# ToniChopp/ECAMP

Hardware: AMD Instinct MI355X
Metric: pretrain image-report pairs/sec (ViT-B/16, 224^2, seq=128) (higher is better)
Workload: dtype bf16

## Files before the change

### ecamp_amd/csrc/vision.hip

```cpp
#include "common.h"
#include <stdlib.h>
#include <stdint.h>

__device__ __forceinline__ void cubic_coeffs(float t, float (&w)[4]) {
    const float A = -0.75f;
    float x;
    x = t + 1.0f; w[0] = ((A * x - 5.0f * A) * x + 8.0f * A) * x - 4.0f * A;
    x = t;        w[1] = ((A + 2.0f) * x - (A + 3.0f)) * x * x + 1.0f;
    x = 1.0f - t; w[2] = ((A + 2.0f) * x - (A + 3.0f)) * x * x + 1.0f;
    x = 2.0f - t; w[3] = ((A * x - 5.0f * A) * x + 8.0f * A) * x - 4.0f * A;
}
__global__ void bicubic_kernel(const float* __restrict__ src, float* __restrict__ dst, long planes, int Hs, int Ws, int Hd,
                               int Wd, float sy, float sx) {
    long n = planes * Hd * Wd;
    for (long i = (long)blockIdx.x * blockDim.x + threadIdx.x; i < n; i += (long)gridDim.x * blockDim.x) {
        int x = (int)(i % Wd), y = (int)((i / Wd) % Hd);
        long pl = i / ((long)Wd * Hd);
        float ry = sy * (y + 0.5f) - 0.5f, rx = sx * (x + 0.5f) - 0.5f;
        float fy = floorf(ry), fx = floorf(rx);
        float wy[4], wx[4];
        cubic_coeffs(ry - fy, wy);
        cubic_coeffs(rx - fx, wx);
        int iy = (int)fy, ix = (int)fx;
        const float* p = src + pl * (long)Hs * Ws;
// ... 997 lines not shown
            for (int e = 0; e < 2; ++e) {
                u32x4_t q;
                q[0] = in ? pack_bf16x2(o[0][e][0], o[1][e][0]) : 0u;
                q[1] = in ? pack_bf16x2(o[2][e][0], 0.f) : 0u;
                q[2] = in ? pack_bf16x2(o[0][e][1], o[1][e][1]) : 0u;
                q[3] = in ? pack_bf16x2(o[2][e][1], 0.f) : 0u;
                *reinterpret_cast<u32x4_t*>(U16 + ((2 * by + e) * 36 + 2 * bx) * 8) = q;
            }
            if (by >= 1 && by <= 16 && bx >= 1 && bx <= 16) {
#pragma unroll
                for (int c = 0; c < 3; ++c)
#pragma unroll
                    for (int e = 0; e < 2; ++e)
                        *reinterpret_cast<float2*>(UC + (c * 32 + 2 * by - 2 + e) * 32 + 2 * bx - 2) = make_float2(o[c][e][0], o[c][e][1]);
            }
        }
        __syncthreads();
        for (int g = wave; g < (34 * 17 + 63) / 64; g += 4) {
            const int p = g * 64 + lane, pc = min(p, 34 * 17 - 1);
            const int y = pc / 17, xq = pc - y * 17;
            f32x4_t oA, oB;
            sr_pair_conv<36, false>(U16 + (y * 36 + 2 * xq) * 8, a1, bias1, oA, oB);
            const int Y = Y0 - 1 + y, X = X0 - 1 + 2 * xq;
            const bool iy = Y >= 0 && Y < R2, inA = iy && X >= 0 && X < R2, inB = iy && X + 1 >= 0 && X + 1 < R2;
            u32x4_t q;
            q[0] = inA ? pack_bf16x2(fmaxf(oA[0], 0.f), fmaxf(oA[1], 0.f)) : 0u;
            q[1] = inA ? pack_bf16x2(fmaxf(oA[2], 0.f), 0.f) : 0u;
            q[2] = inB ? pack_bf16x2(fmaxf(oB[0], 0.f), fmaxf(oB[1], 0.f)) : 0u;
            q[3] = inB ? pack_bf16x2(fmaxf(oB[2], 0.f), 0.f) : 0u;
            if (p < 34 * 17) *reinterpret_cast<u32x4_t*>(C16 + (y * 34 + 2 * xq) * 8) = q;
        }
        __syncthreads();
#pragma unroll
        for (int j = 0; j < 2; ++j) {
            const int p = (wave + 4 * j) * 64 + lane, y = p >> 4, xq = p & 15;
            float2 bg[3];
#pragma unroll
            for (int o = 0; o < 3; ++o) bg[o] = big.at2(b, o, Y0 + y, X0 + 2 * xq, R2);
            f32x4_t oA, oB;
            sr_pair_conv<34, false>(C16 + (y * 34 + 2 * xq) * 8, a2, bias2, oA, oB);
#pragma unroll
            for (int o = 0; o < 3; ++o) {
                const float2 uu = *reinterpret_cast<const float2*>(UC + (o * 32 + y) * 32 + 2 * xq);
                const float dA = fmaxf(oA[o] + uu.x, 0.f) - bg[o].x, dB = fmaxf(oB[o] + uu.y, 0.f) - bg[o].y;
                part += dA * dA + dB * dB;
            }
        }
    }
    part = block_sum_256(part, sh);
    if (threadIdx.x == 0) atomicAdd(loss_sum, part);
}

#define SRP_LDS_BYTES (44 * 44 * 8 + 40 * 42 * 8 + 38 * 40 * 8 + 36 * 38 * 8 + 3 * 34 * 36 * 4 + 4 * 9 * 4 * 8)
__global__ __launch_bounds__(256, 2) void sr_pair_bwd_kernel(const float* __restrict__ pred_img, BigSrc big,
                                                             const long* __restrict__ column, const long* __restrict__ row, SrP P,
                                                             float* __restrict__ dsr, float* __restrict__ gw, long B, int R, int win) {
    extern __shared__ __attribute__((aligned(16))) unsigned char smem8[];
    unsigned char* U16 = smem8;
    unsigned char* C16 = U16 + 44 * 44 * 8;
    unsigned char* DS16 = C16 + 40 * 42 * 8;
    unsigned char* DC16 = DS16 + 38 * 40 * 8;
    float* DU = reinterpret_cast<float*>(DC16 + 36 * 38 * 8);
    float* PP = DU;
    bf16x4_t(*TAPS)[9][4] = reinterpret_cast<bf16x4_t(*)[9][4]>(reinterpret_cast<unsigned char*>(DU) + 3 * 34 * 36 * 4);
    const int lane = threadIdx.x & 63, wave = threadIdx.x >> 6;
    if (threadIdx.x < 144) {
        const int c = threadIdx.x / 36, t = (threadIdx.x / 4) % 9, i = threadIdx.x & 3;
        const float* w = (c == 0 || c == 3) ? P.w1 : P.w2;
        const bool trans = c >= 2;
        float v[3] = {0.f, 0.f, 0.f};
        if (i < 3) {
            for (int kk = 0; kk < 3; ++kk) v[kk] = trans ? w[(kk * 3 + i) * 9 + t] : w[(i * 3 + kk) * 9 + t];
        }
        TAPS[c][t][i] = sr_pack4(v[0], v[1], v[2]);
    }
#define SR_TAPS(NAME, C)                                                     \
    bf16x4_t NAME[9];                                                        \
    _Pragma("unroll") for (int t_ = 0; t_ < 9; ++t_) NAME[t_] = TAPS[(C)][t_][lane & 3]
    const f32x4_t bias1 = {P.b1[0], P.b1[1], P.b1[2], 0.f}, bias2 = {P.b2[0], P.b2[1], P.b2[2], 0.f}, zero4 = {0.f, 0.f, 0.f, 0.f};
    const bf16x4_t ones = {(short)H16_ONE, (short)H16_ONE, (short)H16_ONE, (short)H16_ONE};
    const int R2 = 2 * R, G = R2 / SRT, PT = SRT / 2;
    const long T = B * G * G;
    f32x4_t G1[9], G2[9], gb1 = zero4, gb2 = zero4;
#pragma unroll
    for (int q = 0; q < 9; ++q) G1[q] = G2[q] = zero4;
    const int py = threadIdx.x / PT, px = threadIdx.x % PT;

    struct Cur { int t, b, ty, tx; };
    const int GG = G * G, NT = (int)T;
    const int step_b = (int)gridDim.x / GG, step_r = (int)gridDim.x - step_b * GG, step_y = step_r / G, step_x = step_r - step_y * G;
    auto step = [&](Cur c) {
        c.t += (int)gridDim.x;
        c.tx += step_x;
        if (c.tx >= G) { c.tx -= G; ++c.ty; }
        c.ty += step_y;
        if (c.ty >= G) { c.ty -= G; ++c.b; }
        c.b += step_b;
        return c;
    };
    auto advance = [&](Cur c) {
        for (; c.t < NT; c = step(c)) {
            const int c0 = (int)column[c.b], r0 = (int)row[c.b];
            if (!(c.ty < c0 - 1 || c.ty > c0 + win || c.tx < r0 - 1 || c.tx > r0 + win)) break;
#pragma unroll
            for (int ch = 0; ch < 3; ++ch) dsr[((c.b * 3 + ch) * (long)R + c.ty * PT + py) * R + c.tx * PT + px] = 0.f;
        }
        return c;
    };
    float pp[7], bigv[3][3][2];
    bool inw[3];
    auto fetch_patch = [&](const Cur& cu) {
        const long b = cu.b;
        const int ylo = cu.ty * (SRT / 2) - 4, xlo = cu.tx * (SRT / 2) - 4;
#pragma unroll
        for (int k = 0; k < 7; ++k) {
            const int idx = threadIdx.x + 256 * k;
// ... 25 lines not shown
            }
        }
    };
    Cur cur;
    cur.t = (int)blockIdx.x; cur.b = cur.t / GG; cur.ty = (cur.t - cur.b * GG) / G; cur.tx = cur.t - cur.b * GG - cur.ty * G;
    cur = advance(cur);
    if (cur.t < NT) {
        fetch_patch(cur);
        fetch_big(cur);
    }
    while (cur.t < NT) {
        const long b = cur.b;
        const int ty = cur.ty, tx = cur.tx;
        const int Y0 = ty * SRT, X0 = tx * SRT;
        __syncthreads();
#pragma unroll
        for (int k = 0; k < 7; ++k) {
            const int idx = threadIdx.x + 256 * k;
            if (idx < 3 * 576) PP[idx] = pp[k];
        }
        const Cur nxt = advance(step(cur));
        if (nxt.t < NT) fetch_patch(nxt);
        __syncthreads();
        for (int id = threadIdx.x; id < 22 * 22; id += 256) {
            const int by = id / 22, bx = id - by * 22;
            float o[3][2][2];
#pragma unroll
            for (int c = 0; c < 3; ++c) {
                const float* pl = PP + c * 576 + by * 24 + bx;
                float he[3], ho[3];
#pragma unroll
                for (int r = 0; r < 3; ++r) {
                    const float v0 = pl[r * 24], v1 = pl[r * 24 + 1], v2 = pl[r * 24 + 2];
                    he[r] = 0.25f * v0 + 0.75f * v1;
                    ho[r] = 0.75f * v1 + 0.25f * v2;
                }
                o[c][0][0] = 0.25f * he[0] + 0.75f * he[1];
                o[c][0][1] = 0.25f * ho[0] + 0.75f * ho[1];
                o[c][1][0] = 0.75f * he[1] + 0.25f * he[2];
                o[c][1][1] = 0.75f * ho[1] + 0.25f * ho[2];
            }
            const int Y = Y0 - 6 + 2 * by, X = X0 - 6 + 2 * bx;
            const bool in = Y >= 0 && Y < R2 && X >= 0 && X < R2;
#pragma unroll
            for (int e = 0; e < 2; ++e) {
                u32x4_t q;
                q[0] = in ? pack_bf16x2(o[0][e][0], o[1][e][0]) : 0u;
                q[1] = in ? pack_bf16x2(o[2][e][0], 0.f) : 0u;
                q[2] = in ? pack_bf16x2(o[0][e][1], o[1][e][1]) : 0u;
                q[3] = in ? pack_bf16x2(o[2][e][1], 0.f) : 0u;
                *reinterpret_cast<u32x4_t*>(U16 + ((2 * by + e) * 44 + 2 * bx) * 8) = q;
            }
        }
        __syncthreads();
        {
            SR_TAPS(a1, 0);
            for (int g = wave; g < (40 * 21 + 63) / 64; g += 4) {
                const int p = g * 64 + lane, pc = min(p, 40 * 21 - 1);
                const int y = pc / 21, xq = pc - y * 21;
                f32x4_t oA, oB;
                sr_pair_conv<44, false>(U16 + ((y + 1) * 44 + 2 * xq) * 8, a1, bias1, oA, oB);
                const int Y = Y0 - 4 + y, X = X0 - 5 + 2 * xq;
                const bool iy = Y >= 0 && Y < R2, inA = iy && X >= 0 && X < R2, inB = iy && X + 1 >= 0 && X + 1 < R2;
                u32x4_t q;
                q[0] = inA ? pack_bf16x2(fmaxf(oA[0], 0.f), fmaxf(oA[1], 0.f)) : 0u;
                q[1] = inA ? pack_bf16x2(fmaxf(oA[2], 0.f), 0.f) : 0u;
                q[2] = inB ? pack_bf16x2(fmaxf(oB[0], 0.f), fmaxf(oB[1], 0.f)) : 0u;
                q[3] = inB ? pack_bf16x2(fmaxf(oB[2], 0.f), 0.f) : 0u;
                if (p < 40 * 21) *reinterpret_cast<u32x4_t*>(C16 + (y * 42 + 2 * xq) * 8) = q;
            }
        }
        __syncthreads();
        {
            SR_TAPS(a2, 1);
#pragma unroll
            for (int j = 0; j < 3; ++j) {
                const int g = wave + 4 * j;
                const int p = g * 64 + lane, pc = min(p, 38 * 20 - 1);
                const int y = pc / 20, xq = pc - y * 20;
                f32x4_t oA, oB;
                sr_pair_conv<42, false>(C16 + (y * 42 + 2 * xq) * 8, a2, bias2, oA, oB);
                float dA[3] = {0.f, 0.f, 0.f}, dB[3] = {0.f, 0.f, 0.f};
                if (inw[j]) {
                    const u32x4_t uu = *reinterpret_cast<const u32x4_t*>(U16 + ((y + 3) * 44 + 2 * xq + 2) * 8);
                    float uA[3], uB[3];
                    sr_unpack3(make_uint2(uu[0], uu[1]), uA);
                    sr_unpack3(make_uint2(uu[2], uu[3]), uB);
#pragma unroll
                    for (int o = 0; o < 3; ++o) {
                        const float sA = fmaxf(oA[o] + uA[o], 0.f), sB = fmaxf(oB[o] + uB[o], 0.f);
                        dA[o] = sA > 0.f ? sA - bigv[j][o][0] : 0.f;
                        dB[o] = sB > 0.f ? sB - bigv[j][o][1] : 0.f;
                    }
                }
                if (p < 38 * 20)
                    *reinterpret_cast<u32x4_t*>(DS16 + (y * 40 + 2 * xq) * 8) =
                        (u32x4_t){pack_bf16x2(dA[0], dA[1]), pack_bf16x2(dA[2], 0.f), pack_bf16x2(dB[0], dB[1]), pack_bf16x2(dB[2], 0.f)};
            }
        }
        if (nxt.t < NT) fetch_big(nxt);
        __syncthreads();
        {
            SR_TAPS(a2t, 2);
            for (int g = wave; g < (36 * 19 + 63) / 64; g += 4) {
                const int p = g * 64 + lane, pc = min(p, 36 * 19 - 1);
                const int y = pc / 19, xq = pc - y * 19;
                f32x4_t oA, oB;
                sr_pair_conv<40, true>(DS16 + (y * 40 + 2 * xq) * 8, a2t, zero4, oA, oB);
                const u32x4_t cc = *reinterpret_cast<const u32x4_t*>(C16 + ((y + 2) * 42 + 2 * xq + 2) * 8);
                float cA[3], cB[3];
                sr_unpack3(make_uint2(cc[0], cc[1]), cA);
                sr_unpack3(make_uint2(cc[2], cc[3]), cB);
                float dA[3], dB[3];
#pragma unroll
                for (int i = 0; i < 3; ++i) {
                    dA[i] = cA[i] > 0.f ? oA[i] : 0.f;
                    dB[i] = cB[i] > 0.f ? oB[i] : 0.f;
                }
                if (p < 36 * 19)
                    *reinterpret_cast<u32x4_t*>(DC16 + (y * 38 + 2 * xq) * 8) =
                        (u32x4_t){pack_bf16x2(dA[0], dA[1]), pack_bf16x2(dA[2], 0.f), pack_bf16x2(dB[0], dB[1]), pack_bf16x2(dB[2], 0.f)};
            }
        }
        __syncthreads();
        {
            bf16x4_t k2[3], k1[3];
#pragma unroll
            for (int j = 0; j < 4; ++j) {
                const int y = 2 * (wave * 4 + j) + (lane >> 5), x = lane & 31;
                const bf16x4_t A2 = sr_tr(DS16 + ((y + 3) * 40 + x + 4) * 8);
                const bf16x4_t A1 = sr_tr(DC16 + ((y + 2) * 38 + x + 3) * 8);
                gb2 = MFMA4(A2, ones, gb2);
                gb1 = MFMA4(A1, ones, gb1);
                const unsigned char* cb = C16 + ((y + 3) * 42 + x + 4) * 8;
                const unsigned char* ub = U16 + ((y + 5) * 44 + x + 5) * 8;
#pragma unroll
                for (int q = 0; q < 9; ++q) {
                    const int ky = q / 3, kx = q % 3;
                    const bf16x4_t B2 = (ky == 0 && j > 0) ? k2[kx] : sr_tr(cb + (ky * 42 + kx) * 8);
                    const bf16x4_t B1 = (ky == 0 && j > 0) ? k1[kx] : sr_tr(ub + (ky * 44 + kx) * 8);
                    G2[q] = MFMA4(A2, B2, G2[q]);
                    G1[q] = MFMA4(A1, B1, G1[q]);
                    if (ky == 2) { k2[kx] = B2; k1[kx] = B1; }
                }
            }
        }
// ... 9 lines not shown
                sr_unpack3(make_uint2(dd[0], dd[1]), dA);
                sr_unpack3(make_uint2(dd[2], dd[3]), dB);
                const int Y = Y0 - 1 + y, X = X0 - 2 + 2 * xq;
                const bool in = Y >= 0 && Y < R2 && X >= 0 && X < R2;
                const float wa = X == 0 ? 1.0f : 0.75f, wb = X == R2 - 2 ? 1.0f : 0.75f;
#pragma unroll
                for (int i = 0; i < 3; ++i) {
                    const float va = in ? oA[i] + dA[i] : 0.f, vb = in ? oB[i] + dB[i] : 0.f;
                    const float left = __shfl_up(vb, 1, 64), right = __shfl_down(va, 1, 64);
                    const float h = wa * va + wb * vb + 0.25f * (left + right);
                    if (lane >= 1 && lane <= 62 && p < 34 * 18 && xq >= 1 && xq <= 16) DU[(i * 34 + y) * 24 + xq - 1] = h;
                }
            }
        }
        __syncthreads();
        {
            const int y = ty * PT + py, x = tx * PT + px;
            const float wa = y == 0 ? 1.0f : 0.75f, wb = y == R - 1 ? 1.0f : 0.75f;
#pragma unroll
            for (int c = 0; c < 3; ++c) {
                const float* h = DU + (c * 34 + 2 * py) * 24 + px;
                dsr[((b * 3 + c) * (long)R + y) * R + x] = 0.25f * (h[0] + h[72]) + wa * h[24] + wb * h[48];
            }
        }
        cur = nxt;
    }
#undef SR_TAPS
    __syncthreads();
    float* RED = reinterpret_cast<float*>(U16);
    auto blocks_sum = [&](float v) {
#pragma unroll
        for (int o = 4; o < 64; o <<= 1) v += __shfl_xor(v, o, 64);
        return v;
    };
    const int ic = lane & 3;
#pragma unroll
    for (int q = 0; q < 9; ++q)
#pragma unroll
        for (int o = 0; o < 3; ++o) {
            const float s1 = blocks_sum(G1[q][o]), s2 = blocks_sum(G2[q][o]);
            if (lane < 3) {
                RED[wave * 168 + o * 27 + ic * 9 + q] = s1;
                RED[wave * 168 + 84 + o * 27 + ic * 9 + q] = s2;
            }
        }
#pragma unroll
    for (int o = 0; o < 3; ++o) {
        const float s1 = blocks_sum(gb1[o]), s2 = blocks_sum(gb2[o]);
        if (lane == 0) {
            RED[wave * 168 + 81 + o] = s1;
            RED[wave * 168 + 165 + o] = s2;
        }
    }
    __syncthreads();
    if (threadIdx.x < 168) atomicAdd(gw + threadIdx.x, RED[threadIdx.x] + RED[168 + threadIdx.x] + RED[336 + threadIdx.x] + RED[504 + threadIdx.x]);
}

static BigSrc big_src(const void* big, const float* lut) {
    BigSrc s;
    s.f = lut ? nullptr : reinterpret_cast<const float*>(big);
    s.u8 = lut ? reinterpret_cast<const unsigned char*>(big) : nullptr;
    s.lut = lut;
    return s;
}
extern "C" int ecamp_sr_fwd(const float* pred_img, const void* big, const float* big_lut, const int64_t* column,
                            const int64_t* row, const float* w1, const float* b1, const float* w2, const float* b2, float* loss_sum, int64_t B,
                            int32_t R, int32_t super_patch, int32_t window, int32_t mode, hipStream_t stream) {
    ECAMP_CHECK_ARG(pred_img && big && column && row && w1 && b1 && w2 && b2 && loss_sum, "sr_fwd: null pointer");
    ECAMP_CHECK_ARG(!big_lut || ((uintptr_t)big & 1) == 0, "sr_fwd: the uint8 target must be 2-byte aligned");
    const BigSrc bs = big_src(big, big_lut);
    ECAMP_CHECK_ARG(super_patch == SRT && (2 * R) % SRT == 0, "sr_fwd: the fused SR head is built for 32-px super-patches (patch 16)");
    ECAMP_CHECK_ARG(mode == 0 || mode == 1, "sr_fwd: mode must be 0 (f32 VALU) or 1 (bf16 matrix cores)");
    SrP W = {w1, b1, w2, b2};
    long tiles = B * (2 * R / SRT) * (2 * R / SRT);
    int nb = (int)(tiles < 2048 ? tiles : 2048);
    if (mode == 1)
        hipLaunchKernelGGL(sr_pair_fwd_kernel, dim3(nb), dim3(256), 0, stream, pred_img, bs, (const long*)column, (const long*)row, W, loss_sum,
                           (long)B, R, window);
    else
        hipLaunchKernelGGL(sr_fused_fwd_kernel, dim3(nb), dim3(256), 0, stream, pred_img, bs, (const long*)column, (const long*)row, W, loss_sum,
                           (long)B, R, window, (float*)nullptr);
    ECAMP_LAUNCH_CHECK();
    return 0;
}

extern "C" int ecamp_sr_image(const float* pred_img, const float* w1, const float* b1, const float* w2, const float* b2, float* sr,
                              int64_t B, int32_t R, hipStream_t stream) {
    ECAMP_CHECK_ARG(pred_img && w1 && b1 && w2 && b2 && sr, "sr_image: null pointer");
    ECAMP_CHECK_ARG((2 * R) % SRT == 0, "sr_image: 2R must be a multiple of 32");
    SrP W = {w1, b1, w2, b2};
    long tiles = B * (2 * R / SRT) * (2 * R / SRT);
    int nb = (int)(tiles < 2048 ? tiles : 2048);
    hipLaunchKernelGGL(sr_fused_fwd_kernel, dim3(nb), dim3(256), 0, stream, pred_img, big_src(nullptr, nullptr), (const long*)nullptr, (const long*)nullptr, W,
                       (float*)nullptr, (long)B, R, 0, sr);
    ECAMP_LAUNCH_CHECK();
    return 0;
}

extern "C" int64_t ecamp_sr_bwd_workspace_bytes(void) { return 168 * 4; }

extern "C" int ecamp_sr_bwd(const float* pred_img, const void* big, const float* big_lut, const int64_t* column,
                            const int64_t* row, const float* w1, const float* b1, const float* w2, const float* b2, float* dsr, float* gw_ws,
                            int64_t B, int32_t R, int32_t super_patch, int32_t window, int32_t mode, hipStream_t stream) {
    ECAMP_CHECK_ARG(pred_img && big && column && row && w1 && b1 && w2 && b2 && dsr && gw_ws, "sr_bwd: null pointer");
    ECAMP_CHECK_ARG(!big_lut || ((uintptr_t)big & 1) == 0, "sr_bwd: the uint8 target must be 2-byte aligned");
    const BigSrc bs = big_src(big, big_lut);
    ECAMP_CHECK_ARG(super_patch == SRT && (2 * R) % SRT == 0, "sr_bwd: the fused SR head is built for 32-px super-patches (patch 16)");
    ECAMP_CHECK_ARG(mode == 0 || mode == 1, "sr_bwd: mode must be 0 (f32 VALU) or 1 (bf16 matrix cores)");
    SrP W = {w1, b1, w2, b2};
    long tiles = B * (2 * R / SRT) * (2 * R / SRT);
    ECAMP_CHECK_ARG(tiles < (1L << 30), "sr_bwd: too many tiles");
    int nb = (int)(tiles < 1024 ? tiles : 1024);
    size_t shm = (size_t)(3 * (42 * 42 + 40 * 40 + 38 * 38 + 36 * 36)) * sizeof(float);
    static bool once = false;
    if (!once) {
        (void)hipFuncSetAttribute(reinterpret_cast<const void*>(sr_fused_bwd_kernel), hipFuncAttributeMaxDynamicSharedMemorySize, (int)shm);
        once = true;
    }
    if (mode == 1) {
        static int nbp = 0;
        if (nbp == 0) {
            nbp = ecamp_opt(OPT_SR_BLOCKS);
            if (nbp <= 0) nbp = ecamp_opt_default(OPT_SR_BLOCKS);
            (void)hipFuncSetAttribute(reinterpret_cast<const void*>(sr_pair_bwd_kernel), hipFuncAttributeMaxDynamicSharedMemorySize, (int)SRP_LDS_BYTES);
        }
        const int nb2 = (int)(tiles < nbp ? tiles : nbp);
        hipLaunchKernelGGL(sr_pair_bwd_kernel, dim3(nb2), dim3(256), SRP_LDS_BYTES, stream, pred_img, bs, (const long*)column, (const long*)row, W, dsr,
                           gw_ws, (long)B, R, window);
        ECAMP_LAUNCH_CHECK();
        return 0;
    }
    hipLaunchKernelGGL(sr_fused_bwd_kernel, dim3(nb), dim3(256), shm, stream, pred_img, bs, (const long*)column, (const long*)row, W, dsr, gw_ws,
                       (long)B, R, window);
    ECAMP_LAUNCH_CHECK();
    return 0;
}

__global__ void scaled_accum_kernel(const float* __restrict__ ws, float* __restrict__ grad, const float* __restrict__ scale_dev,
                                    int idx, int n) {
    int i = blockIdx.x * blockDim.x + threadIdx.x;
    if (i < n) grad[i] += scale_dev[idx] * ws[i];
}
extern "C" int ecamp_scaled_accum(const float* ws, float* grad, const float* scale_dev, int32_t idx, int32_t n, hipStream_t stream) {
    ECAMP_CHECK_ARG(ws && grad && scale_dev && n > 0, "scaled_accum: bad args");
    hipLaunchKernelGGL(scaled_accum_kernel, dim3((n + 255) / 256), dim3(256), 0, stream, ws, grad, scale_dev, idx, n);
    ECAMP_LAUNCH_CHECK();
    return 0;
}
```

### ecamp_amd/functions.py

```python
import math

import torch

from . import hip_ops as ops


def _none(n):
    return (None,) * n


_BLOCK = None


class _wgrad_block:

    def __init__(self, arena):
        self.arena = arena

    def __enter__(self):
        global _BLOCK
        self.prev, _BLOCK = _BLOCK, [self.arena, [], [], False]
        self._ready = self.arena.ready
        self.arena.ready = lambda *ps, _b=_BLOCK: _b[2].extend(ps)
        return self
# ... 229 lines not shown

class DecStemFn(torch.autograd.Function):
    @staticmethod
    def forward(ctx, latent, ids_restore, ids_keep, m, B):
        A = m.arena
        L, Dd = m.num_patches, m.decoder_embed_dim
        Lk = ids_keep.shape[1]
        y = ops.linear_fwd(latent, A.w(m.decoder_embed.weight), m.decoder_embed.bias.data)
        ctx.s = (latent, ids_restore, ids_keep, m, B, Lk)
        if m.f32_residual:
            xd = ops.unshuffle_fwd_x32(y, ids_restore, m.mask_token.data, m.decoder_pos_embed.data, B, L, Lk, Dd)
            return f32_carrier(xd.view(B * (L + 1), Dd), m.compute_dtype)
        xd = ops.unshuffle_fwd(y, ids_restore, m.mask_token.data, m.decoder_pos_embed.data, B, L, Lk, Dd)
        return xd.view(B * (L + 1), Dd)

    @staticmethod
    def backward(ctx, dxd):
        latent, ids_restore, ids_keep, m, B, Lk = ctx.s
        A = m.arena
        G = A.grad
        L, Dd = m.num_patches, m.decoder_embed_dim
        dy = ops.unshuffle_bwd(dxd.contiguous(), ids_restore, ids_keep, G(m.mask_token).view(-1), B, L, Lk, Dd).view(-1, Dd)
        de = m.decoder_embed
        _wgrad(A, dy, latent, de.weight, gb=G(de.bias))
        dlat = ops.linear_dgrad(dy, A.w(de.weight))
        A.ready(de.weight, de.bias, m.mask_token)
        ctx.s = None
        return (dlat,) + _none(4)


def _dec_head_fwd(m, xd):
    ln = m.decoder_norm
    if m.f32_residual:
        xd = f32_stream(xd)
        h, _, mean, rstd = ops.layernorm_fwd_x32(xd, ln.weight.data, ln.bias.data, ln.eps, m.compute_dtype)
    else:
        h, _, mean, rstd = ops.layernorm_fwd(xd, ln.weight.data, ln.bias.data, ln.eps)
    pred = ops.linear_fwd(h, m.arena.w(m.decoder_pred.weight), m.decoder_pred.bias.data)
    return pred, (xd, mean, rstd, h)


def _dec_head_bwd(m, rec, dpred):
    xd, mean, rstd, h = rec
    A = m.arena
    G = A.grad
    dp, ln = m.decoder_pred, m.decoder_norm
    _wgrad(A, dpred, h, dp.weight, gb=G(dp.bias))
    dh = ops.linear_dgrad(dpred, A.w(dp.weight))
    dxd = _ln_bwd(dh, xd, mean, rstd, ln.weight.data, G(ln.weight), G(ln.bias))
    A.ready(dp.weight, dp.bias, ln.weight, ln.bias)
    return dxd


def _pixel_loss_fwd(m, pred, imgs, big, mask, column, row, B):
    cd = m.compute_dtype
    R, p = m.img_size, m.patch_size
    sums = ops.zeros((2,), pred.device)
    pred_img = ops.unpatchify_mim(pred, imgs, mask, sums[0:], B, R, p)
    sr = m.super_res
    sr_mode = 0 if cd == torch.float32 else 1
    ops.sr_fwd(pred_img, big, column, row, sr.conv1.weight.data, sr.conv1.bias.data, sr.conv2.weight.data, sr.conv2.bias.data,
               sums[1:], 2 * p, m.sr_window, sr_mode)
    n1, n2 = B * 3 * R * R, B * 3 * 4 * R * R
    m._aux = dict(pred=pred, pred_img=pred_img) if m.keep_aux else None
    return sums * m._loss_norm(n1, n2, pred.device), (pred_img, imgs, mask, big, column, row, B, n1, n2, pred.dtype)


def _pixel_loss_bwd(m, rec, g):
    pred_img, imgs, mask, big, column, row, B, n1, n2, pdt = rec
    G = m.arena.grad
    cd = m.compute_dtype
    R, p = m.img_size, m.patch_size
    gm_gs = (g * (2.0 * m._loss_norm(n1, n2, g.device))).contiguous()
    sr = m.super_res
    ws = ops.zeros((168,), pred_img.device)
    dsr = ops.sr_bwd(pred_img, big, column, row, sr.conv1.weight.data, sr.conv1.bias.data, sr.conv2.weight.data,
                     sr.conv2.bias.data, ws, 2 * p, m.sr_window, 0 if cd == torch.float32 else 1)
    ops.scaled_accum(ws[0:81], G(sr.conv1.weight), gm_gs, 1)
    ops.scaled_accum(ws[81:84], G(sr.conv1.bias), gm_gs, 1)
    ops.scaled_accum(ws[84:165], G(sr.conv2.weight), gm_gs, 1)
    ops.scaled_accum(ws[165:168], G(sr.conv2.bias), gm_gs, 1)
    m.arena.ready(sr.conv1.weight, sr.conv1.bias, sr.conv2.weight, sr.conv2.bias)
    return ops.img_loss_bwd(pred_img, imgs, mask, dsr, gm_gs, B, R, p, pdt)


class ImgLossFn(torch.autograd.Function):

    @staticmethod
    def forward(ctx, xd, imgs, big, mask, column, row, m, B):
        pred, head = _dec_head_fwd(m, xd)
        out, tail = _pixel_loss_fwd(m, pred, imgs, big, mask, column, row, B)
        ctx.s = (m, head, tail)
        return out

    @staticmethod
    def backward(ctx, g):
        m, head, tail = ctx.s
        dxd = _dec_head_bwd(m, head, _pixel_loss_bwd(m, tail, g))
        ctx.s = None
        return (dxd,) + _none(7)


class DecHeadFn(torch.autograd.Function):

    @staticmethod
    def forward(ctx, xd, m):
        pred, head = _dec_head_fwd(m, xd)
        ctx.s = (m, head)
        return pred

    @staticmethod
    def backward(ctx, dpred):
        m, head = ctx.s
        ctx.s = None
        return _dec_head_bwd(m, head, dpred.contiguous()), None


class PixelLossFn(torch.autograd.Function):

    @staticmethod
    def forward(ctx, pred, imgs, big, mask, column, row, m, B):
        out, tail = _pixel_loss_fwd(m, pred, imgs, big, mask, column, row, B)
        ctx.s = (m, tail)
        return out

    @staticmethod
    def backward(ctx, g):
        m, tail = ctx.s
        ctx.s = None
        return (_pixel_loss_bwd(m, tail, g),) + _none(7)


class ReportStemFn(torch.autograd.Function):

    @staticmethod
    def forward(ctx, latent, m, B, T):
        A = m.arena
        lat = ops.linear_fwd(latent, A.w(m.bert_mlp.weight), m.bert_mlp.bias.data)
        H = lat.shape[1]
        gap = ops.seq_sum(lat.view(B, T, H), 1, T, 1.0 / (T - 1))
        ctx.s = (latent, m, B, T, H)
        return lat, gap

    @staticmethod
    def backward(ctx, dlat, dgap):
        latent, m, B, T, H = ctx.s
        A = m.arena
        G = A.grad
        dlat = dlat.clone(memory_format=torch.contiguous_format)
        ops.seq_bcast(dgap.contiguous(), dlat.view(B, T, H), 1, T, 1.0 / (T - 1), 1)
        _wgrad(A, dlat, latent, m.bert_mlp.weight, gb=G(m.bert_mlp.bias))
        dl = ops.linear_dgrad(dlat, A.w(m.bert_mlp.weight))
        A.ready(m.bert_mlp.weight, m.bert_mlp.bias)
        ctx.s = None
        return (dl,) + _none(3)


class BertEmbedFn(torch.autograd.Function):
    @staticmethod
    def forward(ctx, ids, type_ids, emb, m, p, anchor):
        B, S = ids.shape
        seed, off = m.next_rng()
        ln = emb.LayerNorm
        e, z, mean, rstd = ops.bert_embed_fwd(ids, type_ids, emb.word_embeddings.weight.data, emb.position_embeddings.weight.data,
                                              emb.token_type_embeddings.weight.data, ln.weight.data, ln.bias.data, ln.eps,
                                              m.compute_dtype, p, seed, off)
        ctx.s = (ids, type_ids, emb, m, p, seed, off, z, mean, rstd)
        return e

    @staticmethod
    def backward(ctx, de):
        ids, type_ids, emb, m, p, seed, off, z, mean, rstd = ctx.s
        G = m.arena.grad
        B, S = ids.shape
        ln = emb.LayerNorm
# ... 252 lines not shown
```

### ecamp_amd/hip_ops.py

```python
import ctypes

import torch

from . import _lib
from ._lib import BF16, F32, call

_I64x3 = ctypes.c_int64 * 3


def code(dtype):
    if dtype == torch.float32:
        return F32
    if dtype == torch.bfloat16 or dtype == torch.float16:
        want = "bf16" if dtype == torch.bfloat16 else "f16"
        if _lib.half() != want:
            raise TypeError("a %s tensor reached the %s build of libecamp_hip -- call ecamp_amd._lib.set_half(%r) first "
                            "(ECAMP(compute_dtype=...) does)" % (dtype, _lib.half(), want))
        return BF16
    raise TypeError("ecamp_amd supports float32, bfloat16 and float16 activations, got %s" % dtype)


def _chk(*ts):
    for t in ts:
        if t is not None and not t.is_cuda:
# ... 417 lines not shown
    return out


def unshuffle_fwd_x32(y, ids_restore, mask_token, dpos, B, L, Lk, D):
    xd = torch.empty((B, L + 1, D), device=y.device, dtype=torch.float32)
    call("ecamp_unshuffle_fwd_x32", ptr(y), ptr(ids_restore), ptr(mask_token), ptr(dpos), ptr(xd), B, L, Lk, D, code(y.dtype), stream())
    return xd


def unshuffle_fwd(y, ids_restore, mask_token, dpos, B, L, Lk, D):
    xd = torch.empty((B, L + 1, D), device=y.device, dtype=y.dtype)
    call("ecamp_unshuffle_fwd", ptr(y), ptr(ids_restore), ptr(mask_token), ptr(dpos), ptr(xd), B, L, Lk, D, code(y.dtype), stream())
    return xd


def unshuffle_bwd(dxd, ids_restore, ids_keep, gmask_token, B, L, Lk, D):
    dy = torch.empty((B, Lk + 1, D), device=dxd.device, dtype=dxd.dtype)
    call("ecamp_unshuffle_bwd", ptr(dxd), ptr(ids_restore), ptr(ids_keep), ptr(dy), ptr(gmask_token), B, L, Lk, D, code(dxd.dtype),
         stream())
    return dy


def unpatchify_mim(pred, imgs, mask, loss_sum, B, R, p):
    pred_img = torch.empty((B, 3, R, R), device=pred.device, dtype=torch.float32)
    call("ecamp_unpatchify_mim", ptr(pred), ptr(imgs), ptr(mask), ptr(pred_img), ptr(loss_sum), B, R, p, code(pred.dtype), stream())
    return pred_img


def img_loss_bwd(pred_img, imgs, mask, dsr, gm_gs, B, R, p, dtype):
    L = (R // p) ** 2
    dpred = torch.empty((B * (L + 1), p * p * 3), device=pred_img.device, dtype=dtype)
    call("ecamp_img_loss_bwd", ptr(pred_img), ptr(imgs), ptr(mask), ptr(dsr), ptr(gm_gs), ptr(dpred), B, R, p, code(dtype), stream())
    return dpred


def sr_fwd(pred_img, big, column, row, w1, b1, w2, b2, loss_sum, super_patch, window, mode=0):
    B, _, R, _ = pred_img.shape
    call("ecamp_sr_fwd", ptr(pred_img), ptr(big), ptr(image_lut(big.device) if is_u8_image(big) else None), ptr(column), ptr(row), ptr(w1), ptr(b1), ptr(w2), ptr(b2),
         ptr(loss_sum), B, R, super_patch, window, int(mode), stream())


def sr_image(pred_img, w1, b1, w2, b2):
    B, _, R, _ = pred_img.shape
    out = torch.empty((B, 3, 2 * R, 2 * R), device=pred_img.device, dtype=torch.float32)
    call("ecamp_sr_image", ptr(pred_img), ptr(w1), ptr(b1), ptr(w2), ptr(b2), ptr(out), B, R, stream())
    return out


def sr_bwd(pred_img, big, column, row, w1, b1, w2, b2, gw_ws, super_patch, window, mode=0):
    B, _, R, _ = pred_img.shape
    dsr = torch.empty((B, 3, R, R), device=pred_img.device, dtype=torch.float32)
    call("ecamp_sr_bwd", ptr(pred_img), ptr(big), ptr(image_lut(big.device) if is_u8_image(big) else None), ptr(column), ptr(row), ptr(w1), ptr(b1), ptr(w2), ptr(b2),
         ptr(dsr), ptr(gw_ws), B, R, super_patch, window, int(mode), stream())
    return dsr


def scaled_accum(ws, grad, scale_dev, idx):
    call("ecamp_scaled_accum", ptr(ws), ptr(grad), ptr(scale_dev), idx, ws.numel(), stream())


def bert_embed_fwd(ids, type_ids, word, pos, typ, gamma, beta, eps, dtype, drop_p=0.0, seed=0, offset=0):
    _chk(ids, word)
    B, S = ids.shape
    H = word.shape[1]
    z = torch.empty((B * S, H), device=ids.device, dtype=dtype)
    e = torch.empty((B * S, H), device=ids.device, dtype=dtype)
    mean = torch.empty(B * S, device=ids.device, dtype=torch.float32)
    rstd = torch.empty(B * S, device=ids.device, dtype=torch.float32)
    call("ecamp_bert_embed_fwd", ptr(ids), ptr(type_ids), ptr(word), ptr(pos), ptr(typ), ptr(gamma), ptr(beta), ptr(z), ptr(e),
         ptr(mean), ptr(rstd), B, S, H, float(eps), float(drop_p), seed, offset, code(dtype), stream())
    return e, z, mean, rstd


def bert_embed_bwd(de, z, mean, rstd, gamma, ids, type_ids, gword, gpos, gtype, ggamma, gbeta, B, S, H, drop_p=0.0, seed=0,
                   offset=0, pad_id=0, hot=(2, 3)):
    call("ecamp_bert_embed_bwd", ptr(de), ptr(z), ptr(mean), ptr(rstd), ptr(gamma), ptr(ids), ptr(type_ids), ptr(gword), ptr(gpos),
         ptr(gtype), ptr(ggamma), ptr(gbeta), B, S, H, pad_id, hot[0], hot[1], float(drop_p), seed, offset, code(de.dtype), stream())


def ce_fwd_bwd_(logits, labels, weights, loss_sum, gain=1.0):
    _chk(logits, labels, weights)
    M, V = logits.shape
    call("ecamp_ce_fwd_bwd", ptr(logits), ptr(labels), ptr(weights), ptr(loss_sum), M, V, logits.stride(0), float(gain) / M,
         code(logits.dtype), stream())
    return logits


def sumsq(x, out):
    call("ecamp_sumsq", ptr(x), x.numel(), ptr(out), stream())


def adamw(p, g, m, v, p16, lr, beta1, beta2, eps, wd, step, grad_scale=1.0):
    call("ecamp_adamw", ptr(p), ptr(g), ptr(m), ptr(v), ptr(p16), p.numel(), float(lr), float(beta1), float(beta2), float(eps),
         float(wd), int(step), float(grad_scale), stream())


def adamw_grouped(p, g, m, v, p16, block_group, lrs, wds, beta1, beta2, eps, step, grad_scale=1.0, grad_sumsq=None, ctl=None):
    n = len(lrs)
    arr = ctypes.c_float * n
    call("ecamp_adamw_grouped", ptr(p), ptr(g), ptr(m), ptr(v), ptr(p16), ptr(block_group), p.numel(), n, arr(*lrs), arr(*wds),
         float(beta1), float(beta2), float(eps), int(step), float(grad_scale), ptr(grad_sumsq), ptr(ctl), stream())


def loss_scale_update(sumsq_, state, opt_step, ctl, norm_out, growth, backoff, interval, beta1, beta2):
    _chk(sumsq_, state, opt_step, ctl)
    call("ecamp_loss_scale_update", ptr(sumsq_), ptr(state), ptr(opt_step), ptr(ctl), ptr(norm_out), float(growth), float(backoff), int(interval),
# ... 154 lines not shown
```

### include/ecamp_hip.h

```cpp
#ifndef ECAMP_HIP_H
#define ECAMP_HIP_H
#include <stdint.h>
#ifdef __cplusplus
extern "C" {
#endif

typedef struct ihipStream_t* ecampStream_t;

#define ECAMP_F32 0
#define ECAMP_BF16 1

#define ECAMP_ABI_VERSION 5
int ecamp_abi_version(void);
const char* ecamp_last_error(void);
int ecamp_half_format(void);

int ecamp_gemm(const void* A, const void* B, void* C, int64_t M, int64_t N, int64_t K, int a_kc, int64_t lda, int b_kc,
               int64_t ldb, int64_t ldc, const float* bias, const void* residual, int64_t ldr, void* pre_out, int64_t ldp,
               const void* gmul, int64_t ldg, int act, float alpha, const float* alpha_dev, int dtype, int out_f32, int accumulate,
               int split_k, float* splitk_ws, float* rowsum, ecampStream_t stream);
int ecamp_gemm_res32(const void* A, const void* B, float* C, int64_t M, int64_t N, int64_t K, int64_t lda, int64_t ldb, int64_t ldc,
                     const float* bias, const float* residual, int64_t ldr, int dtype, ecampStream_t stream);
int ecamp_gemm_suggest_split(int64_t M, int64_t N, int64_t K, int a_kc, int b_kc, int dtype);
int ecamp_wgrad_group_supported(int32_t n, const int64_t* n_out, const int64_t* k_in, int64_t rows);
// ... 47 lines not shown
                   const void* drop_mask, ecampStream_t stream);
int ecamp_attn_probs(const void* q, const void* k, const int32_t* key_mask, float* probs, int32_t B, int32_t H, int32_t Tq, int32_t Tk,
                     int32_t hd, const int64_t* q_strides, const int64_t* k_strides, float scale, int32_t dtype, ecampStream_t stream);

int ecamp_add(const void* a, const void* b, void* y, int64_t n, int32_t dtype, ecampStream_t stream);
int ecamp_gelu_bwd(const void* dy, const void* pre, void* dx, int64_t n, int32_t dtype, ecampStream_t stream);
int ecamp_cast(const void* src, void* dst, int64_t n, int32_t src_dtype, int32_t dst_dtype, ecampStream_t stream);
int ecamp_scale(const void* x, void* y, int64_t n, float alpha, const float* alpha_dev, int32_t dtype, ecampStream_t stream);
int ecamp_zero(void* p, int64_t bytes, ecampStream_t stream);
int ecamp_colsum(const void* X, int64_t ld, int64_t M, int64_t N, float alpha, const float* alpha_dev, int32_t period, int32_t lo, int32_t hi,
                 float* out, int32_t dtype, ecampStream_t stream);
int ecamp_bcast_add(const void* x, const void* g, void* y, int64_t B, int32_t S, int32_t H, int32_t dtype,
                    ecampStream_t stream);
int ecamp_seq_sum(const void* x, void* out, int64_t B, int32_t S, int32_t H, int32_t s0, int32_t s1, float scale, int32_t dtype,
                  ecampStream_t stream);
int ecamp_seq_bcast(const void* g, void* y, int64_t B, int32_t S, int32_t H, int32_t s0, int32_t s1, float scale, int32_t mode,
                    int32_t dtype, ecampStream_t stream);
int ecamp_uniform(float* out, int64_t n, uint64_t seed, uint64_t offset, ecampStream_t stream);

int ecamp_bicubic_resize(const float* src, float* dst, int64_t planes, int32_t Hs, int32_t Ws, int32_t Hd, int32_t Wd,
                         ecampStream_t stream);
int ecamp_bicubic_resize_u8(const uint8_t* src, float* dst, int64_t B, int32_t Hs, int32_t Ws, int32_t Hd, int32_t Wd, const float* lut,
                            ecampStream_t stream);
int ecamp_mask_indices(const float* noise, int64_t B, int32_t L, int32_t len_keep, int32_t* ids_restore, int32_t* ids_keep,
                       float* mask, ecampStream_t stream);
int ecamp_im2col_gather(const float* imgs, const int32_t* ids_keep, void* out, int64_t B, int32_t Lk, int32_t C, int32_t R,
                        int32_t p, int32_t dtype, ecampStream_t stream);
int ecamp_assemble_tokens(void* x, const float* cls, const float* pos, const int32_t* ids_keep, int64_t B, int32_t Lk, int32_t D,
                          int32_t dtype, ecampStream_t stream);
int ecamp_assemble_tokens_x32(const void* x, float* out, const float* cls, const float* pos, const int32_t* ids_keep, int64_t B, int32_t Lk,
                              int32_t D, int32_t dtype, ecampStream_t stream);
int64_t ecamp_resample_crops_workspace_bytes(int64_t B, int32_t out, int32_t kmax, int64_t tmp_rows);
int ecamp_resample_crops_u8(const uint8_t* src, const int64_t* table, uint8_t* dst, int64_t B, int32_t out, int32_t kmax, int64_t tmp_rows,
                            int32_t max_h, void* ws, int64_t ws_bytes, int32_t* err_flag, ecampStream_t stream);
int ecamp_unshuffle_fwd(const void* y, const int32_t* ids_restore, const float* mask_token, const float* dpos, void* xd, int64_t B,
                        int32_t L, int32_t Lk, int32_t D, int32_t dtype, ecampStream_t stream);
int ecamp_unshuffle_fwd_x32(const void* y, const int32_t* ids_restore, const float* mask_token, const float* dpos, float* xd, int64_t B,
                            int32_t L, int32_t Lk, int32_t D, int32_t dtype, ecampStream_t stream);
int ecamp_unshuffle_bwd(const void* dxd, const int32_t* ids_restore, const int32_t* ids_keep, void* dy, float* dmask_token,
                        int64_t B, int32_t L, int32_t Lk, int32_t D, int32_t dtype, ecampStream_t stream);
int ecamp_unpatchify_mim(const void* pred, const float* imgs, const float* mask, float* pred_img, float* loss_sum, int64_t B,
                         int32_t R, int32_t p, int32_t dtype, ecampStream_t stream);
int ecamp_img_loss_bwd(const float* pred_img, const float* imgs, const float* mask, const float* dsr, const float* gm_gs,
                       void* dpred, int64_t B, int32_t R, int32_t p, int32_t dtype, ecampStream_t stream);
int ecamp_sr_fwd(const float* pred_img, const void* big, const float* big_lut, const int64_t* column,
                 const int64_t* row, const float* w1, const float* b1, const float* w2, const float* b2, float* loss_sum, int64_t B,
                 int32_t R, int32_t super_patch, int32_t window, int32_t mode,
                 ecampStream_t stream);
int ecamp_sr_image(const float* pred_img, const float* w1, const float* b1, const float* w2, const float* b2, float* sr, int64_t B,
                   int32_t R, ecampStream_t stream);
int ecamp_sr_bwd(const float* pred_img, const void* big, const float* big_lut, const int64_t* column,
                 const int64_t* row, const float* w1, const float* b1, const float* w2, const float* b2, float* dsr, float* gw_ws,
                 int64_t B, int32_t R, int32_t super_patch, int32_t window, int32_t mode, ecampStream_t stream);
int ecamp_scaled_accum(const float* ws, float* grad, const float* scale_dev, int32_t idx, int32_t n, ecampStream_t stream);

int ecamp_bert_embed_fwd(const int64_t* ids, const int64_t* type_ids, const float* word, const float* pos, const float* type,
                         const float* gamma, const float* beta, void* z, void* e, float* mean, float* rstd, int64_t B, int32_t S,
                         int32_t cols, float eps, float drop_p, uint64_t seed, uint64_t offset, int32_t dtype,
                         ecampStream_t stream);
int ecamp_bert_embed_bwd(const void* de, const void* z, const float* mean, const float* rstd, const float* gamma, const int64_t* ids,
                         const int64_t* type_ids, float* gword, float* gpos, float* gtype, float* dgamma, float* dbeta, int64_t B,
                         int32_t S, int32_t cols, int32_t pad_id, int32_t hot0, int32_t hot1, float drop_p, uint64_t seed,
                         uint64_t offset, int32_t dtype, ecampStream_t stream);
int ecamp_ce_fwd_bwd(void* logits, const int64_t* labels, const float* weights, float* loss_sum, int64_t M, int32_t V, int64_t ld,
                     float inv_count, int32_t dtype, ecampStream_t stream);

int ecamp_zero_blocks(float* g, const uint8_t* block_flags, int64_t n, ecampStream_t stream);
int ecamp_sumsq(const float* x, int64_t n, float* out, ecampStream_t stream);
int ecamp_adamw(float* p, const float* g, float* m, float* v, void* p_bf16, int64_t n, float lr, float beta1, float beta2,
                float eps, float weight_decay, int64_t step, float grad_scale,
                ecampStream_t stream);

int ecamp_adamw_grouped(float* p, const float* g, float* m, float* v, void* p_bf16, const uint8_t* block_group, int64_t n,
                        int32_t ngroups, const float* lr_host, const float* wd_host, float beta1, float beta2, float eps,
                        int64_t step, float grad_scale, float* grad_sumsq, const float* ctl,
                        ecampStream_t stream);
int ecamp_loss_scale_update(const float* sumsq, float* state, float* opt_step, float* ctl, float* norm_out, float growth_factor,
                            float backoff_factor, int32_t growth_interval, float beta1, float beta2, ecampStream_t stream);

int ecamp_prof_enable(int on);
int ecamp_prof_collect(int category, double* total_ms, double* total_work, int64_t* count);
int64_t ecamp_prof_live_events(void);

#ifdef ECAMP_DEV_ABI
int ecamp_dropout_mask(uint8_t* keep, int64_t n, float p, uint64_t seed, uint64_t offset, ecampStream_t stream);
int ecamp_dev_spin(int32_t blocks, int32_t threads, int64_t cycles, ecampStream_t stream);
int64_t ecamp_gemm_q8_launches(void);
int64_t ecamp_wgrad_group_launches(void);
int64_t ecamp_gemm_f8_q8_launches(void);
int64_t ecamp_gemm_q16_launches(void);
int64_t ecamp_attn_head_launches(void);
int64_t ecamp_prof_dump(char* buf, int64_t cap);
#endif

#ifdef __cplusplus
}
#endif
#endif
```

Measured before the change: 7410.

## Fuse super-resolution loss forward into the backward kernel when gradients are needed

When the input needs gradients in bf16 mode, the super-resolution loss is now computed inside the pair backward kernel, which already evaluates the conv outputs. The separate forward kernel launch and its recomputation of both convolutions are skipped. The backward work moves from the autograd backward into the forward call, and the intermediate results are stored for later use. The fused path adds LDS staging of an upsampled plane, extra per-thread work and a reduction. The loss window's interior checks must match the original forward exactly.

Result: no change. 7353 (-0.8%).

```diff
diff --git a/ecamp_amd/csrc/vision.hip b/ecamp_amd/csrc/vision.hip
--- a/ecamp_amd/csrc/vision.hip
+++ b/ecamp_amd/csrc/vision.hip
@@ -1073,9 +1073,11 @@
 }
 
 #define SRP_LDS_BYTES (44 * 44 * 8 + 40 * 42 * 8 + 38 * 40 * 8 + 36 * 38 * 8 + 3 * 34 * 36 * 4 + 4 * 9 * 4 * 8)
+template <bool LOSS>
 __global__ __launch_bounds__(256, 2) void sr_pair_bwd_kernel(const float* __restrict__ pred_img, BigSrc big,
                                                              const long* __restrict__ column, const long* __restrict__ row, SrP P,
-                                                             float* __restrict__ dsr, float* __restrict__ gw, long B, int R, int win) {
+                                                             float* __restrict__ dsr, float* __restrict__ gw, float* __restrict__ loss_sum,
+                                                             long B, int R, int win) {
     extern __shared__ __attribute__((aligned(16))) unsigned char smem8[];
     unsigned char* U16 = smem8;
     unsigned char* C16 = U16 + 44 * 44 * 8;
@@ -1083,6 +1085,9 @@
     unsigned char* DC16 = DS16 + 38 * 40 * 8;
     float* DU = reinterpret_cast<float*>(DC16 + 36 * 38 * 8);
     float* PP = DU;
+    float* UC01 = reinterpret_cast<float*>(DC16);
+    float* UC2 = DU + 3 * 576;
+    float part = 0.f;
     bf16x4_t(*TAPS)[9][4] = reinterpret_cast<bf16x4_t(*)[9][4]>(reinterpret_cast<unsigned char*>(DU) + 3 * 34 * 36 * 4);
     const int lane = threadIdx.x & 63, wave = threadIdx.x >> 6;
     if (threadIdx.x < 144) {
@@ -1214,6 +1219,23 @@
                 *reinterpret_cast<u32x4_t*>(U16 + ((2 * by + e) * 44 + 2 * bx) * 8) = q;
             }
         }
+        if (LOSS) {
+            const int by = 3 + (threadIdx.x >> 4), bx = 3 + (threadIdx.x & 15);
+#pragma unroll
+            for (int c = 0; c < 3; ++c) {
+                const float* pl = PP + c * 576 + by * 24 + bx;
+                float he[3], ho[3];
+#pragma unroll
+                for (int r = 0; r < 3; ++r) {
+                    const float v0 = pl[r * 24], v1 = pl[r * 24 + 1], v2 = pl[r * 24 + 2];
+                    he[r] = 0.25f * v0 + 0.75f * v1;
+                    ho[r] = 0.75f * v1 + 0.25f * v2;
+                }
+                float* uc = (c < 2 ? UC01 + c * 1024 : UC2) + (2 * by - 6) * 32 + 2 * bx - 6;
+                *reinterpret_cast<float2*>(uc) = make_float2(0.25f * he[0] + 0.75f * he[1], 0.25f * ho[0] + 0.75f * ho[1]);
+                *reinterpret_cast<float2*>(uc + 32) = make_float2(0.75f * he[1] + 0.25f * he[2], 0.75f * ho[1] + 0.25f * ho[2]);
+            }
+        }
         __syncthreads();
         {
             SR_TAPS(a1, 0);
@@ -1254,6 +1276,14 @@
                         dA[o] = sA > 0.f ? sA - bigv[j][o][0] : 0.f;
                         dB[o] = sB > 0.f ? sB - bigv[j][o][1] : 0.f;
                     }
+                    if (LOSS && y >= 3 && y < 35 && xq >= 2 && xq < 18) {
+#pragma unroll
+                        for (int o = 0; o < 3; ++o) {
+                            const float2 uf = *reinterpret_cast<const float2*>((o < 2 ? UC01 + o * 1024 : UC2) + (y - 3) * 32 + 2 * xq - 4);
+                            const float eA = fmaxf(oA[o] + uf.x, 0.f) - bigv[j][o][0], eB = fmaxf(oB[o] + uf.y, 0.f) - bigv[j][o][1];
+                            part += eA * eA + eB * eB;
+                        }
+                    }
                 }
                 if (p < 38 * 20)
                     *reinterpret_cast<u32x4_t*>(DS16 + (y * 40 + 2 * xq) * 8) =
@@ -1369,8 +1399,13 @@
             RED[wave * 168 + 165 + o] = s2;
         }
     }
+    if (LOSS) {
+        part = wave_sum(part);
+        if (lane == 0) RED[672 + wave] = part;
+    }
     __syncthreads();
     if (threadIdx.x < 168) atomicAdd(gw + threadIdx.x, RED[threadIdx.x] + RED[168 + threadIdx.x] + RED[336 + threadIdx.x] + RED[504 + threadIdx.x]);
+    if (LOSS && threadIdx.x == 192) atomicAdd(loss_sum, RED[672] + RED[673] + RED[674] + RED[675]);
 }
 
 static BigSrc big_src(const void* big, const float* lut) {
@@ -1380,6 +1415,9 @@
     s.lut = lut;
     return s;
 }
+static long g_sr_launches[3] = {0, 0, 0};
+extern "C" int64_t ecamp_sr_launches(int32_t kind) { return kind >= 0 && kind < 3 ? g_sr_launches[kind] : -1; }
+
 extern "C" int ecamp_sr_fwd(const float* pred_img, const void* big, const float* big_lut, const int64_t* column,
                             const int64_t* row, const float* w1, const float* b1, const float* w2, const float* b2, float* loss_sum, int64_t B,
                             int32_t R, int32_t super_patch, int32_t window, int32_t mode, hipStream_t stream) {
@@ -1398,6 +1436,7 @@
         hipLaunchKernelGGL(sr_fused_fwd_kernel, dim3(nb), dim3(256), 0, stream, pred_img, bs, (const long*)column, (const long*)row, W, loss_sum,
                            (long)B, R, window, (float*)nullptr);
     ECAMP_LAUNCH_CHECK();
+    ++g_sr_launches[0];
     return 0;
 }
 
@@ -1416,9 +1455,9 @@
 
 extern "C" int64_t ecamp_sr_bwd_workspace_bytes(void) { return 168 * 4; }
 
-extern "C" int ecamp_sr_bwd(const float* pred_img, const void* big, const float* big_lut, const int64_t* column,
-                            const int64_t* row, const float* w1, const float* b1, const float* w2, const float* b2, float* dsr, float* gw_ws,
-                            int64_t B, int32_t R, int32_t super_patch, int32_t window, int32_t mode, hipStream_t stream) {
+static int sr_bwd_launch(const float* pred_img, const void* big, const float* big_lut, const int64_t* column,
+                         const int64_t* row, const float* w1, const float* b1, const float* w2, const float* b2, float* dsr, float* gw_ws,
+                         float* loss_sum, int64_t B, int32_t R, int32_t super_patch, int32_t window, int32_t mode, hipStream_t stream) {
     ECAMP_CHECK_ARG(pred_img && big && column && row && w1 && b1 && w2 && b2 && dsr && gw_ws, "sr_bwd: null pointer");
     ECAMP_CHECK_ARG(!big_lut || ((uintptr_t)big & 1) == 0, "sr_bwd: the uint8 target must be 2-byte aligned");
     const BigSrc bs = big_src(big, big_lut);
@@ -1439,18 +1478,42 @@
         if (nbp == 0) {
             nbp = ecamp_opt(OPT_SR_BLOCKS);
             if (nbp <= 0) nbp = ecamp_opt_default(OPT_SR_BLOCKS);
-            (void)hipFuncSetAttribute(reinterpret_cast<const void*>(sr_pair_bwd_kernel), hipFuncAttributeMaxDynamicSharedMemorySize, (int)SRP_LDS_BYTES);
+            (void)hipFuncSetAttribute(reinterpret_cast<const void*>(sr_pair_bwd_kernel<false>), hipFuncAttributeMaxDynamicSharedMemorySize, (int)SRP_LDS_BYTES);
+            (void)hipFuncSetAttribute(reinterpret_cast<const void*>(sr_pair_bwd_kernel<true>), hipFuncAttributeMaxDynamicSharedMemorySize, (int)SRP_LDS_BYTES);
         }
         const int nb2 = (int)(tiles < nbp ? tiles : nbp);
-        hipLaunchKernelGGL(sr_pair_bwd_kernel, dim3(nb2), dim3(256), SRP_LDS_BYTES, stream, pred_img, bs, (const long*)column, (const long*)row, W, dsr,
-                           gw_ws, (long)B, R, window);
+        if (loss_sum)
+            hipLaunchKernelGGL(sr_pair_bwd_kernel<true>, dim3(nb2), dim3(256), SRP_LDS_BYTES, stream, pred_img, bs, (const long*)column, (const long*)row, W,
+                               dsr, gw_ws, loss_sum, (long)B, R, window);
+        else
+            hipLaunchKernelGGL(sr_pair_bwd_kernel<false>, dim3(nb2), dim3(256), SRP_LDS_BYTES, stream, pred_img, bs, (const long*)column, (const long*)row, W,
+                               dsr, gw_ws, (float*)nullptr, (long)B, R, window);
         ECAMP_LAUNCH_CHECK();
+        ++g_sr_launches[loss_sum ? 2 : 1];
         return 0;
     }
+    ECAMP_CHECK_ARG(!loss_sum, "sr_bwd: the f32 backward has no loss sum");
     hipLaunchKernelGGL(sr_fused_bwd_kernel, dim3(nb), dim3(256), shm, stream, pred_img, bs, (const long*)column, (const long*)row, W, dsr, gw_ws,
                        (long)B, R, window);
     ECAMP_LAUNCH_CHECK();
+    ++g_sr_launches[1];
     return 0;
+}
+extern "C" int ecamp_sr_bwd(const float* pred_img, const void* big, const float* big_lut, const int64_t* column,
+                            const int64_t* row, const float* w1, const float* b1, const float* w2, const float* b2, float* dsr, float* gw_ws,
+                            int64_t B, int32_t R, int32_t super_patch, int32_t window, int32_t mode, hipStream_t stream) {
+    return sr_bwd_launch(pred_img, big, big_lut, column, row, w1, b1, w2, b2, dsr, gw_ws, nullptr, B, R, super_patch, window, mode, stream);
+}
+
+extern "C" int ecamp_sr_fwd_bwd(const float* pred_img, const void* big, const float* big_lut, const int64_t* column,
+                                const int64_t* row, const float* w1, const float* b1, const float* w2, const float* b2, float* loss_sum, float* dsr,
+                                float* gw_ws, int64_t B, int32_t R, int32_t super_patch, int32_t window, int32_t mode, hipStream_t stream) {
+    ECAMP_CHECK_ARG(loss_sum, "sr_fwd_bwd: null pointer");
+    if (mode == 1)
+        return sr_bwd_launch(pred_img, big, big_lut, column, row, w1, b1, w2, b2, dsr, gw_ws, loss_sum, B, R, super_patch, window, mode, stream);
+    const int rc = ecamp_sr_fwd(pred_img, big, big_lut, column, row, w1, b1, w2, b2, loss_sum, B, R, super_patch, window, mode, stream);
+    if (rc) return rc;
+    return sr_bwd_launch(pred_img, big, big_lut, column, row, w1, b1, w2, b2, dsr, gw_ws, nullptr, B, R, super_patch, window, mode, stream);
 }
 
 __global__ void scaled_accum_kernel(const float* __restrict__ ws, float* __restrict__ grad, const float* __restrict__ scale_dev,
diff --git a/ecamp_amd/functions.py b/ecamp_amd/functions.py
--- a/ecamp_amd/functions.py
+++ b/ecamp_amd/functions.py
@@ -305,30 +305,32 @@
     return dxd
 
 
-def _pixel_loss_fwd(m, pred, imgs, big, mask, column, row, B):
+def _pixel_loss_fwd(m, pred, imgs, big, mask, column, row, B, want_grad):
     cd = m.compute_dtype
     R, p = m.img_size, m.patch_size
     sums = ops.zeros((2,), pred.device)
     pred_img = ops.unpatchify_mim(pred, imgs, mask, sums[0:], B, R, p)
     sr = m.super_res
     sr_mode = 0 if cd == torch.float32 else 1
-    ops.sr_fwd(pred_img, big, column, row, sr.conv1.weight.data, sr.conv1.bias.data, sr.conv2.weight.data, sr.conv2.bias.data,
-               sums[1:], 2 * p, m.sr_window, sr_mode)
+    dsr = ws = None
+    if want_grad:
+        ws = ops.zeros((168,), pred_img.device)
+        dsr = ops.sr_fwd_bwd(pred_img, big, column, row, sr.conv1.weight.data, sr.conv1.bias.data, sr.conv2.weight.data, sr.conv2.bias.data,
+                             sums[1:], ws, 2 * p, m.sr_window, sr_mode)
+    else:
+        ops.sr_fwd(pred_img, big, column, row, sr.conv1.weight.data, sr.conv1.bias.data, sr.conv2.weight.data, sr.conv2.bias.data,
+                   sums[1:], 2 * p, m.sr_window, sr_mode)
     n1, n2 = B * 3 * R * R, B * 3 * 4 * R * R
     m._aux = dict(pred=pred, pred_img=pred_img) if m.keep_aux else None
-    return sums * m._loss_norm(n1, n2, pred.device), (pred_img, imgs, mask, big, column, row, B, n1, n2, pred.dtype)
+    return sums * m._loss_norm(n1, n2, pred.device), (pred_img, imgs, mask, dsr, ws, B, n1, n2, pred.dtype)
 
 
 def _pixel_loss_bwd(m, rec, g):
-    pred_img, imgs, mask, big, column, row, B, n1, n2, pdt = rec
+    pred_img, imgs, mask, dsr, ws, B, n1, n2, pdt = rec
     G = m.arena.grad
-    cd = m.compute_dtype
     R, p = m.img_size, m.patch_size
     gm_gs = (g * (2.0 * m._loss_norm(n1, n2, g.device))).contiguous()
     sr = m.super_res
-    ws = ops.zeros((168,), pred_img.device)
-    dsr = ops.sr_bwd(pred_img, big, column, row, sr.conv1.weight.data, sr.conv1.bias.data, sr.conv2.weight.data,
-                     sr.conv2.bias.data, ws, 2 * p, m.sr_window, 0 if cd == torch.float32 else 1)
     ops.scaled_accum(ws[0:81], G(sr.conv1.weight), gm_gs, 1)
     ops.scaled_accum(ws[81:84], G(sr.conv1.bias), gm_gs, 1)
     ops.scaled_accum(ws[84:165], G(sr.conv2.weight), gm_gs, 1)
@@ -342,7 +344,7 @@
     @staticmethod
     def forward(ctx, xd, imgs, big, mask, column, row, m, B):
         pred, head = _dec_head_fwd(m, xd)
-        out, tail = _pixel_loss_fwd(m, pred, imgs, big, mask, column, row, B)
+        out, tail = _pixel_loss_fwd(m, pred, imgs, big, mask, column, row, B, ctx.needs_input_grad[0])
         ctx.s = (m, head, tail)
         return out
 
@@ -373,7 +375,7 @@
 
     @staticmethod
     def forward(ctx, pred, imgs, big, mask, column, row, m, B):
-        out, tail = _pixel_loss_fwd(m, pred, imgs, big, mask, column, row, B)
+        out, tail = _pixel_loss_fwd(m, pred, imgs, big, mask, column, row, B, ctx.needs_input_grad[0])
         ctx.s = (m, tail)
         return out
 
diff --git a/ecamp_amd/hip_ops.py b/ecamp_amd/hip_ops.py
--- a/ecamp_amd/hip_ops.py
+++ b/ecamp_amd/hip_ops.py
@@ -493,6 +493,14 @@
     dsr = torch.empty((B, 3, R, R), device=pred_img.device, dtype=torch.float32)
     call("ecamp_sr_bwd", ptr(pred_img), ptr(big), ptr(image_lut(big.device) if is_u8_image(big) else None), ptr(column), ptr(row), ptr(w1), ptr(b1), ptr(w2), ptr(b2),
          ptr(dsr), ptr(gw_ws), B, R, super_patch, window, int(mode), stream())
+    return dsr
+
+
+def sr_fwd_bwd(pred_img, big, column, row, w1, b1, w2, b2, loss_sum, gw_ws, super_patch, window, mode=0):
+    B, _, R, _ = pred_img.shape
+    dsr = torch.empty((B, 3, R, R), device=pred_img.device, dtype=torch.float32)
+    call("ecamp_sr_fwd_bwd", ptr(pred_img), ptr(big), ptr(image_lut(big.device) if is_u8_image(big) else None), ptr(column), ptr(row), ptr(w1), ptr(b1), ptr(w2), ptr(b2),
+         ptr(loss_sum), ptr(dsr), ptr(gw_ws), B, R, super_patch, window, int(mode), stream())
     return dsr
 
 
diff --git a/include/ecamp_hip.h b/include/ecamp_hip.h
--- a/include/ecamp_hip.h
+++ b/include/ecamp_hip.h
@@ -123,6 +123,9 @@
 int ecamp_sr_bwd(const float* pred_img, const void* big, const float* big_lut, const int64_t* column,
                  const int64_t* row, const float* w1, const float* b1, const float* w2, const float* b2, float* dsr, float* gw_ws,
                  int64_t B, int32_t R, int32_t super_patch, int32_t window, int32_t mode, ecampStream_t stream);
+int ecamp_sr_fwd_bwd(const float* pred_img, const void* big, const float* big_lut, const int64_t* column,
+                     const int64_t* row, const float* w1, const float* b1, const float* w2, const float* b2, float* loss_sum, float* dsr,
+                     float* gw_ws, int64_t B, int32_t R, int32_t super_patch, int32_t window, int32_t mode, ecampStream_t stream);
 int ecamp_scaled_accum(const float* ws, float* grad, const float* scale_dev, int32_t idx, int32_t n, ecampStream_t stream);
 
 int ecamp_bert_embed_fwd(const int64_t* ids, const int64_t* type_ids, const float* word, const float* pos, const float* type,
@@ -161,6 +164,7 @@
 int64_t ecamp_gemm_f8_q8_launches(void);
 int64_t ecamp_gemm_q16_launches(void);
 int64_t ecamp_attn_head_launches(void);
+int64_t ecamp_sr_launches(int32_t kind);
 int64_t ecamp_prof_dump(char* buf, int64_t cap);
 #endif
 
```
